# uber-research/UPSNet

Measured on AMD Instinct MI355X. Metric: images/sec (whole node), UPSNet-50 1024x2048, higher is better.
Workload: dtype f32

## Files before the change

include/upsnet_hip.h:

```cpp
#ifndef UPSNET_HIP_H
#define UPSNET_HIP_H

#include <stddef.h>
#include <stdint.h>

#ifdef __cplusplus
extern "C" {
#endif

const char *upsnet_last_error(void);
const char *upsnet_last_kernel_form(void);
int upsnet_abi_version(void);

int upsnet_zero_fill(void *stream, void *ptr, size_t bytes);


int upsnet_roi_align_forward(void *stream, const float *bottom_data, float spatial_scale, int num_rois,
                             int height, int width, int channels, int pooled_height, int pooled_width,
                             int sampling_ratio, const float *bottom_rois, float *top_data);

int upsnet_roi_align_forward_nhwc(void *stream, const float *feat_nhwc, int batch, int height, int width,
                                  int channels, float spatial_scale, const float *rois, int num_rois,
                                  int pooled_height, int pooled_width, int sampling_ratio, float *out_nhwc);

// ... 114 lines not shown

int upsnet_conv2d_nhwc_bf16(void *stream, int nseg, const float *const x[], const float *const residual[], float *const out[],
                            const int batch[], const int height[], const int width[], int Cin, const void *wpack_hi,
                            const void *wpack_lo, int ldw, const float *bias, int Cout, int KH, int KW, int stride, int pad,
                            int relu);
int upsnet_conv_pack_weight_bf16(void *stream, const float *weight, int cout, int cin, int kh, int kw, int ldw, void *wpack_hi,
                                 void *wpack_lo);
int upsnet_bottleneck_proj_bf16(void *stream, const void *x, void *out, int batch, int height_in, int width_in, int cin, int cmid, int stride,
                                const void *w1, const void *w2, const void *w3d, const float *b1, const float *b2, const float *b3d);
int upsnet_conv_bf16_tuning(int enable, int tile_rows);
int upsnet_conv1x1_bf16_tuning(int enable);
int upsnet_stem_pool_pack_weight_f32(void *stream, const float *weight, int cin, float *wpack);
int upsnet_stem_pool_f32(void *stream, const float *x4, int batch, int height, int width, const float *wpack, const float *bias, float *out);
int upsnet_stem_pool_pack_weight_bf16(void *stream, const float *weight, int cin, void *wpack);
int upsnet_stem_pool_bf16(void *stream, const float *x4, int batch, int height, int width, const void *wpack, const float *bias, void *out);
int upsnet_deconv2x2_nhwc_bf16(void *stream, const void *x, int batch, int height, int width, int Cin, const void *wpack_hi, int ldw,
                               const float *bias, int Cout, int relu, void *out, int out_bf16);

int upsnet_bottleneck_bf16(void *stream, const void *x, void *out, int batch, int height, int width, int cmid, const void *w1,
                           const void *w2, const void *w3, const float *b1, const float *b2, const float *b3);

int upsnet_conv2d_stem_nhwc4_f32(void *stream, const float *x, int batch, int height, int width, const float *wpack,
                                 int ldw, const float *bias, int Cout, int KH, int KW, int stride, int pad, int relu,
                                 float *out);
int upsnet_conv_pack_weight_stem(void *stream, const float *weight, int cout, int cin, int kh, int kw, int ldw, float *wpack);

int upsnet_deconv2x2_nhwc_f32(void *stream, const float *x, int batch, int height, int width, int Cin, const float *wpack,
                              int ldw, const float *bias, int Cout, int relu, float *out);
int upsnet_deconv2x2_pack_weight(void *stream, const float *weight, int cin, int cout, int ldw, float *wpack);

int upsnet_deconv2x2_frag_nhwc_f32(void *stream, const float *x, float *out, int batch, int height, int width, int Cin,
                                   const float *wpack, const float *bias4, int Cout, int relu);

void upsnet_conv_tuning(int winograd_tiles, int force_tile);

int upsnet_conv_pack_weight(void *stream, const float *weight, int cout, int cin, int kh, int kw, int ldw, float *wpack);

int upsnet_conv1x1_frag_nhwc_f32(void *stream, const float *x, const float *residual, float *out, int batch, int height, int width,
                                 int Cin, const float *wpack, const float *bias, int Cout, int stride, int relu, int residual_up);
void upsnet_conv1x1_tuning(int bn);
int upsnet_conv1x1_siblings_nhwc_f32(void *stream, const float *x, float *out_a, float *out_b, int batch, int height, int width, int Cin,
                                     const float *wpack, const float *bias, int cout_a, int cout_b, int stride, int relu_a, int relu_b);
void upsnet_conv1x1_pair32_tuning(int waves);

int upsnet_residency_tuning(int kernel, int cap);
size_t upsnet_residency_pad_bytes(int cap, size_t static_lds, size_t dynamic_lds);
int upsnet_residency_last_dynamic_lds(void);

int upsnet_conv2d_winograd36_nhwc_f32(void *stream, int nseg, const float *const x[], float *const out[], const int batch[],
                                      const int height[], const int width[], int Cin, const float *wpack, int ldw, const float *bias,
                                      int Cout, int relu);
int upsnet_conv_pack_weight_winograd36(void *stream, const float *weight, int cout, int cin, int ldw, float *wpack);
size_t upsnet_conv2d_winograd36_splitk_workspace_bytes(int batch, int height, int width, int Cout, int ksplit);
int upsnet_conv2d_winograd36_nhwc_f32_splitk(void *stream, const float *x, float *out, int batch, int height, int width, int Cin,
                                             const float *wpack, int ldw, const float *bias, int Cout, int relu, int ksplit, void *workspace);

size_t upsnet_conv1x1_ksw_packed_weight_floats(int cout, int cin);
int upsnet_conv1x1_ksw_pack_weight(void *stream, const float *weight, int cout, int cin, float *wpack);
int upsnet_conv1x1_ksw_nhwc_f32(void *stream, const float *x, const float *residual, float *out, int batch, int height, int width, int Cin,
                                const float *wpack, const float *bias, int Cout, int stride, int relu, int tile_pixels, int tile_channels,
                                int split_n);
void upsnet_conv1x1_ksw_tuning(int tile);

size_t upsnet_conv3x3_ksw_packed_weight_floats(int cin);
int upsnet_conv3x3_ksw_pack_weight(void *stream, const float *weight, int cout, int cin, float *wpack);
int upsnet_conv3x3_ksw_nhwc_f32(void *stream, const float *x, float *out, int batch, int height, int width, int Cin, const float *wpack,
// ... 337 lines not shown
```

upsnet_amd/_lib.py:

```python
import ctypes
import os

import torch

_HERE = os.path.dirname(os.path.abspath(__file__))
LIB_PATH = os.environ.get("UPSNET_LIB_PATH") or os.path.join(_HERE, "csrc", "libupsnet_hip.so")

c_int, c_float, c_double, c_void_p, c_size_t, c_long = ctypes.c_int, ctypes.c_float, ctypes.c_double, ctypes.c_void_p, ctypes.c_size_t, ctypes.c_long
P = c_void_p

_SIGNATURES = {
    "upsnet_last_error": (ctypes.c_char_p, []),
    "upsnet_last_kernel_form": (ctypes.c_char_p, []),
    "upsnet_abi_version": (c_int, []),
    "upsnet_zero_fill": (c_int, [P, P, c_size_t]),
    "upsnet_roi_align_forward": (c_int, [P, P, c_float, c_int, c_int, c_int, c_int, c_int, c_int, c_int, P, P]),
    "upsnet_roi_align_forward_nhwc": (c_int, [P, P, c_int, c_int, c_int, c_int, c_float, P, c_int, c_int, c_int, c_int, P]),
    "upsnet_fpn_roi_align_forward": (c_int, [P, P, P, P, P, c_int, P, c_int, P, c_int, c_int, c_int, P, P]),
    "upsnet_fpn_roi_order": (c_int, [P, P, c_int, P, c_int, c_int, P]),
    "upsnet_fpn_roi_align_forward_ordered": (c_int, [P, P, P, P, P, c_int, P, c_int, P, c_int, c_int, c_int, P, P, P]),
    "upsnet_roi_tuning": (None, [c_int]),
    "upsnet_roi_geometry": (None, [c_int, c_int]),
    "upsnet_deform_im2col": (c_int, [P, P, P] + [c_int] * 13 + [P]),
    "upsnet_mod_deform_im2col": (c_int, [P, P, P, P] + [c_int] * 15 + [P]),
# ... 36 lines not shown
    "upsnet_conv_tuning": (None, [c_int, c_int]),
    "upsnet_conv_pack_weight": (c_int, [P, P, c_int, c_int, c_int, c_int, c_int, P]),
    "upsnet_nms_host": (c_int, [P, P, P, c_int, c_int, c_float, c_int]),
    "upsnet_nms_workspace_bytes": (c_size_t, [c_int, c_int]),
    "upsnet_nms_batched": (c_int, [P, P, P, P, P, c_int, c_int, c_float, P, P, P]),
    "upsnet_nms_tuning": (None, [c_int]),
    "upsnet_cpu_nms_batched": (c_int, [P, P, P, P, c_int, c_int, c_double, P, P, P]),
    "upsnet_soft_nms_batched_workspace_bytes": (c_size_t, [c_int, c_int]),
    "upsnet_soft_nms_batched": (c_int, [P, P, P, P, c_int, c_int, c_float, c_float, c_float, c_int, P, P]),
    "upsnet_soft_nms_workspace_bytes": (c_size_t, [c_int]),
    "upsnet_soft_nms": (c_int, [P, P, P, c_int, c_float, c_float, c_float, c_int, P, P]),
    "upsnet_proposal_workspace_bytes": (c_size_t, [c_int, P, P, c_int, c_int, c_int]),
    "upsnet_pyramid_proposals_strided": (c_int, [P, c_int, P, P, P, P, P, P, P, P, P, P, c_int, P, c_int, c_int, c_float, c_float, P, P, P, P]),
    "upsnet_pyramid_proposals_strided_ordered": (c_int, [P, c_int, P, P, P, P, P, P, P, P, P, P, c_int, P, c_int, c_int, c_float, c_float, P, P, P, P, P]),
    "upsnet_pyramid_proposals_joint_strided": (c_int, [P, c_int, P, P, P, P, P, P, P, P, P, P, c_int, P, c_int, c_int, c_float, c_float, P, P, P, P]),
    "upsnet_pyramid_proposals": (c_int, [P, c_int, P, P, P, P, P, P, c_int, P, c_int, c_int, c_float, c_float, P, P, P, P]),
    "upsnet_mask_roi_capacity": (c_int, [c_int, c_int, c_int]),
    "upsnet_mask_roi_workspace_bytes": (c_size_t, [c_int, c_int, c_int]),
    "upsnet_mask_roi": (c_int, [P, P, P, P, c_int, P, c_int, P, c_int, c_float, c_float, c_int, P, P, P, P, P, P, P]),
    "upsnet_mask_roi_ex": (c_int, [P, P, P, P, c_int, P, c_int, P, c_int, c_int, c_float, c_float, c_int, P, P, P, P, P, P, P]),
    "upsnet_mask_logit_gather": (c_int, [P, P, c_int, c_int, c_int, c_long, c_long, c_long, P, P, c_int, P]),
    "upsnet_mask_removal_workspace_bytes": (c_size_t, [c_int, c_int, c_int, c_int]),
    "upsnet_mask_removal": (c_int, [P, P, P, P, P, c_int, P, c_int, c_int, c_int, c_int, c_double, P, P, P, P]),
    "upsnet_panoptic_tail_pack": (c_int, [P, P, P, c_int, P, P, P, P, P, P, P, P]),
    "upsnet_mask_paste": (c_int, [P, P, P, P, P, P, c_int, c_int, c_int, c_int, P]),
    "upsnet_seg_term": (c_int, [P, P, c_int, c_int, c_int, P, P, P, c_int, P]),
    "upsnet_panoptic_fuse": (c_int, [P, P, c_int, c_int, c_int, c_int, P, P, P, P, P, P, c_int, c_int, P, c_int, P, P]),
    "upsnet_panoptic_fuse_up": (c_int, [P, P, c_int, c_int, c_int, c_int, c_int, c_int, P, P, P, P, P, P, c_int, c_int, P, P, P]),
    "upsnet_conv2d_stem_nhwc4_f32": (c_int, [P, P, c_int, c_int, c_int, P, c_int, P, c_int, c_int, c_int, c_int, c_int, c_int, P]),
    "upsnet_conv_pack_weight_stem": (c_int, [P, P, c_int, c_int, c_int, c_int, c_int, P]),
    "upsnet_deconv2x2_nhwc_f32": (c_int, [P, P, c_int, c_int, c_int, c_int, P, c_int, P, c_int, c_int, P]),
    "upsnet_deconv2x2_pack_weight": (c_int, [P, P, c_int, c_int, c_int, P]),
    "upsnet_deconv2x2_frag_nhwc_f32": (c_int, [P, P, P, c_int, c_int, c_int, c_int, P, P, c_int, c_int]),
    "upsnet_prep_image_u8": (c_int, [P, P, c_int, c_int, P, c_double, c_int, c_int, c_int, c_int, c_int, P]),
    "upsnet_image_to_nhwc4": (c_int, [P, P, c_int, c_int, c_int, c_int, P]),
    "upsnet_unified_pan_workspace_bytes": (c_size_t, []),
    "upsnet_unified_pan_result": (c_int, [P, P, P, P, c_int, c_int, c_int, c_int, c_int, c_int, P, P]),
    "upsnet_combined_pan_workspace_bytes": (c_size_t, [c_int, c_long]),
    "upsnet_combined_pan_result": (c_int, [P, c_int, P, c_int, c_int, c_long, P, P, c_int, c_int, c_int, c_double, P]),
    "upsnet_mask_roi_dedup": (c_int, [P, P, P, P, c_int, P, P, P, P, c_int, P, P, P]),
    "upsnet_conv2d_winograd_nhwc_f32": (c_int, [P, c_int, P, P, P, P, P, P, c_int, P, c_int, P, c_int, c_int]),
    "upsnet_conv2d_winograd_nhwc_f32_splitk": (c_int, [P, P, P, P, c_int, c_int, c_int, c_int, P, c_int, P, c_int, c_int, c_int, P]),
    "upsnet_conv_pack_weight_winograd": (c_int, [P, P, c_int, c_int, c_int, P]),
    "upsnet_conv_pack_weight_winograd_tn32": (c_int, [P, P, c_int, c_int, c_int, P]),
    "upsnet_conv2d_winograd_nhwc_f32_tn32": (c_int, [P, c_int, P, P, P, P, P, P, c_int, P, c_int, P, c_int, c_int]),
    "upsnet_conv2d_winograd_nhwc_f32_tail": (c_int, [P, P, P, c_int, c_int, c_int, c_int, c_int, P, c_int, P, c_int, P, c_int, c_int]),
    "upsnet_conv2d_winograd36_nhwc_f32": (c_int, [P, c_int, P, P, P, P, P, c_int, P, c_int, P, c_int, c_int]),
    "upsnet_conv_pack_weight_winograd36": (c_int, [P, P, c_int, c_int, c_int, P]),
    "upsnet_conv2d_nhwc_bf16": (c_int, [P, c_int, P, P, P, P, P, P, c_int, P, P, c_int, P, c_int, c_int, c_int, c_int, c_int, c_int]),
    "upsnet_bottleneck_proj_bf16": (c_int, [P, P, P, c_int, c_int, c_int, c_int, c_int, c_int, P, P, P, P, P, P]),
    "upsnet_conv_bf16_tuning": (c_int, [c_int, c_int]),
    "upsnet_conv1x1_bf16_tuning": (c_int, [c_int]),
    "upsnet_stem_pool_pack_weight_f32": (c_int, [P, P, c_int, P]),
    "upsnet_stem_pool_f32": (c_int, [P, P, c_int, c_int, c_int, P, P, P]),
    "upsnet_stem_pool_pack_weight_bf16": (c_int, [P, P, c_int, P]),
    "upsnet_stem_pool_bf16": (c_int, [P, P, c_int, c_int, c_int, P, P, P]),
    "upsnet_deconv2x2_nhwc_bf16": (c_int, [P, P, c_int, c_int, c_int, c_int, P, c_int, P, c_int, c_int, P, c_int]),
    "upsnet_bottleneck_bf16": (c_int, [P, P, P, c_int, c_int, c_int, c_int, P, P, P, P, P, P]),
    "upsnet_conv_pack_weight_bf16": (c_int, [P, P, c_int, c_int, c_int, c_int, c_int, P, P]),
    "upsnet_conv2d_splitk_workspace_bytes": (c_size_t, [c_int, c_int, c_int, c_int, c_int, c_int, c_int, c_int, c_int]),
    "upsnet_conv2d_nhwc_f32_splitk": (c_int, [P, P, P, P, c_int, c_int, c_int, c_int, P, c_int, P, c_int, c_int, c_int, c_int, c_int, c_int, c_int, P]),
    "upsnet_im_post_rle": (c_int, [P, P, P, P, c_int, c_int, c_int, c_int, c_int, c_int, P, P]),
    "upsnet_fcn_score_combine": (c_int, [P, c_int, P, c_int, c_int, c_int, P, P]),
    "upsnet_panoptic_argmax": (c_int, [P, P, c_int, c_int, c_int, c_int, P, P, c_int, c_int, P]),
    "upsnet_pq_workspace_bytes": (c_size_t, [c_int]),
    "upsnet_pq_accumulate": (c_int, [P, P, P, c_int, c_int, P, c_int, P, c_int, c_int, P, P, P, P, P, P]),
# ... 140 lines not shown
```

upsnet_amd/build.py:

```python
import hashlib
import os
import re
import subprocess
import sys

HERE = os.path.dirname(os.path.abspath(__file__))
CSRC = os.path.join(HERE, "csrc")
INCLUDE = os.path.join(os.path.dirname(HERE), "include")
LIB = os.path.join(CSRC, "libupsnet_hip.so")
STAMP = LIB + ".srchash"
SOURCES = ["capi.cpp", "fill.hip", "roi_align.hip", "nms.hip", "deform_conv.hip", "deform_fused.hip", "deform_fused_bf16.hip", "backward.hip", "conv.hip", "conv1x1.hip", "conv1x1_ksw.hip", "conv1x1_pair.hip", "conv_wino.hip", "conv_wino36.hip", "conv_bf16.hip", "bottleneck_bf16.hip", "conv3x3_wreg_bf16.hip", "conv1x1_wreg_bf16.hip", "stem_pool_bf16.hip", "stem_pool.hip", "proposal.hip", "detect.hip", "panoptic.hip", "fcn_head.hip", "preprocess.hip", "postprocess.hip", "pq_eval.hip", "pq_boundary.hip", "det_eval.hip", "poly_raster.hip", "restore.hip", "pan_combine.hip", "prop_eval.hip", "cs_inst_eval.hip", "cs_pixel_eval.hip", "pan_format.hip", "vis_render.hip", "pan_vis.hip", "gt_prepare.hip", "group_norm.hip", "cs_inst_format.hip", "tta.hip", "box_vote.hip", "pan_track.hip", "video_eval.hip", "mots_eval.hip", "pan_components.hip"]
FLAGS = ["--offload-arch=gfx950", "-O3", "-ffp-contract=off", "-fno-slp-vectorize", "-std=c++17", "-fPIC", "-Wall", "-Wno-unused-function"]


_COMMENT = re.compile(rb"//[^\n]*|/\*.*?\*/", re.S)


def _source_hash():
    h = hashlib.sha1(" ".join(FLAGS + SOURCES).encode())
    deps = sorted(os.path.join(CSRC, f) for f in os.listdir(CSRC) if f.endswith((".hip", ".cpp", ".h")))
    deps.append(os.path.join(INCLUDE, "upsnet_hip.h"))
    for d in deps:
        h.update(os.path.basename(d).encode())
        with open(d, "rb") as f:
            h.update(b" ".join(_COMMENT.sub(b" ", f.read()).split()))
    return h.hexdigest()


def _stale():
    if not os.path.exists(LIB) or not os.path.exists(STAMP):
        return True
    with open(STAMP) as f:
        return f.read().strip() != _source_hash()


def build(force=False, verbose=True):
    if not force and not _stale():
        return LIB
    hipcc = os.environ.get("HIPCC", "hipcc")
    objs = []
    procs = []
    for src in SOURCES:
        obj = os.path.join(CSRC, os.path.splitext(src)[0] + ".o")
        cmd = [hipcc] + FLAGS + ["-I" + INCLUDE, "-I" + CSRC, "-x", "hip", "-c", os.path.join(CSRC, src), "-o", obj]
# ... 19 lines not shown
```

upsnet_amd/knobs.py:

```python
import os
import re

_ROOT = os.path.dirname(os.path.abspath(__file__))
_NAME = re.compile(r'UPSNET_[A-Z0-9_]+')

REGISTRY = {
    'UPSNET_ALLOW_LIBRARY_CONV': ('0', 'models/hipconv.py', 'a convolution no hand-written kernel covers runs on the library instead of raising'),
    'UPSNET_BF16_ACT': ('1', 'models/hipconv.py', 'bf16 mode: bf16 activations between the layers (0: fp32 activations)'),
    'UPSNET_BF16_BLOCK': ('1', 'models/hipconv.py', 'bf16 mode: one-launch bottlenecks (0: three launches)'),
    'UPSNET_BF16_BLOCK_MIN_TILES': ('128', 'models/hipconv.py', 'bf16 mode: fewest tiles for the one-launch bottleneck'),
    'UPSNET_BF16_HALO': ('1', 'csrc/conv_bf16.hip', 'bf16 3x3 layers on the haloed-patch kernel (0: general kernel)'),
    'UPSNET_BF16_MIN_WG': ('192', 'models/hipconv.py', 'bf16 mode: fewest workgroups for a bf16 layer'),
    'UPSNET_BF16_MIN_WG_WREG': ('16', 'models/hipconv.py', 'bf16 mode: fewest workgroups for the weights-from-L2 3x3 kernel'),
    'UPSNET_BF16_NARROW_BELOW': ('384', 'csrc/conv_bf16.hip', 'bf16 general kernel: 128 x 64 tiles below this many workgroups'),
    'UPSNET_BF16_PROJ': ('1', 'models/hipconv.py', 'bf16 mode: projection bottlenecks as one launch'),
    'UPSNET_BF16_STEM': ('1', 'models/hipconv.py', 'bf16 mode: fused stem + pool kernel'),
    'UPSNET_BF16_WREG': ('1', 'csrc/conv3x3_wreg_bf16.hip', 'bf16 3x3 layers on the weights-from-L2 kernel'),
    'UPSNET_BF16_WREG1': ('1', 'csrc/conv1x1_wreg_bf16.hip', 'bf16 1x1 layers on the no-LDS kernel where it wins'),
    'UPSNET_BF16_WREG_TH': ('auto', 'csrc/conv3x3_wreg_bf16.hip', 'tile rows of the weights-from-L2 3x3 kernel'),
    'UPSNET_CONV1X1': ('1', 'models/hipconv.py', '1x1 layers on the lean GEMM kernel (0: implicit-GEMM kernel)'),
    'UPSNET_CONV1X1_BALANCE': ('0', 'models/hipconv.py', 'split-K tail for unevenly tiled 1x1 layers'),
    'UPSNET_CONV1X1_MIN_WG': ('256', 'models/hipconv.py', 'fewest workgroups for the lean 1x1 kernel'),
    'UPSNET_CONV1X1_KSW': ('1', 'models/hipconv.py', 'small-tile (16x16x4 fragment) 1x1 kernel for maps the 64-pixel tiles do not fill evenly'),
    'UPSNET_CONV1X1_KSW_MAX_FILL': ('0.75', 'models/hipconv.py', 'use it when the last round of 64-pixel workgroups is less than this full'),
    'UPSNET_CONV3X3_KSW': ('1', 'models/hipconv.py', 'small-tile 3x3 kernel for <= 32-channel layers (offset predictors) on small maps'),
    'UPSNET_CONV1X1_PAIR': ('1', 'models/hipconv.py', 'conv3 + next conv1 in one launch'),
    'UPSNET_CONV1X1_PAIR32_WAVES': ('8', 'ops.py', 'waves per workgroup of the res4 pair kernel'),
    'UPSNET_CONV1X1_PAIR_MIN_TILES': ('1024', 'models/hipconv.py', 'fewest tiles for the res2 pair kernel'),
    'UPSNET_CONV1X1_PAIR_RES3': ('1', 'models/hipconv.py', 'pair kernel on res3'),
    'UPSNET_CONV1X1_PAIR_RES4': ('1', 'models/hipconv.py', 'pair kernel on res4'),
    'UPSNET_CONV1X1_SIBLINGS': ('1', 'models/hipconv.py', 'conv1 + projection shortcut in one launch'),
    'UPSNET_CONV_PRECISION': ('fp32', 'models/hipconv.py', 'fp32 | bf16 | bf16x3 (bench.py --conv-precision)'),
    'UPSNET_DCN_BF16': ('1', 'ops.py', 'bf16 mode: fused deformable convolution on the bf16 cores'),
    'UPSNET_DCN_KERNEL': ('frag', 'ops.py', 'generation of the fused deformable kernel'),
    'UPSNET_DCN_SMALL_GRID': ('0', 'csrc/deform_fused.hip', 'small-grid variant threshold of the fused deformable kernel'),
    'UPSNET_DCN_SPLITK': ('1', 'ops.py', 'split-K for the offset predictors of small maps'),
    'UPSNET_DCN_VARIANT': ('5', 'csrc/deform_fused.hip', 'schedule variant of the fused deformable kernel'),
    'UPSNET_DECONV_FRAG': ('1', 'models/hipconv.py', 'transposed convolution on the lean GEMM kernel'),
    'UPSNET_DIST_BACKEND': ('nccl', 'upsnet_end2end_test.py', 'torch.distributed backend of the harness (gloo when ranks share a GPU)'),
    'UPSNET_EARLY_MASK': ('1', 'models/resnet_upsnet.py', 'mask head on the side stream as soon as the detections exist'),
    'UPSNET_FC_RELU': ('1', 'models/rcnn.py', 'ReLU of fc6 / fc7 in the library GEMM epilogue (0: separate elementwise launch)'),
    'UPSNET_GRAPH': ('1', 'models/resnet_upsnet.py', 'whole forward as one HIP graph'),
    'UPSNET_GRAPH_ALIAS': ('1', 'models/resnet_upsnet.py', 'outputs are views into the graph buffers (0: copies)'),
    'UPSNET_GRAPH_OWN_STREAM': ('0', 'models/resnet_upsnet.py', 'capture / replay on an own stream with one instance'),
    'UPSNET_GRAPH_SLOTS': ('2', 'models/resnet_upsnet.py', 'graph instances per input shape'),
    'UPSNET_HIP_MEMSET': ('0', 'csrc/fill.hip', 'zero scratch with hipMemsetAsync instead of a kernel'),
    'UPSNET_LIB_PATH': ('', '_lib.py', 'path of libupsnet_hip.so (same-box A/B of two builds)'),
    'UPSNET_NMS_LDS': ('0', 'csrc/nms.hip', 'stage the suppression mask in LDS'),
    'UPSNET_NMS_SCAN16': ('1', 'csrc/nms.hip', 'unrolled scan for <= 1024 boxes'),
    'UPSNET_OVERLAP': ('1', 'models/resnet_upsnet.py', 'semantic branch on a side stream'),
    'UPSNET_PIN': ('1', 'upsnet_end2end_test.py', 'pin each rank to its CPU slice'),
    'UPSNET_ROI_KERNEL': ('auto', 'csrc/roi_align.hip', 'ROIAlign kernel variant 0..4; auto = 3 (corner-sharing) for >= 100 bins per ROI, else 0 -- so '
                                                        '"0" is NOT the default; upsnet_roi_tuning(v >= 0) overrides the variable, (v < 0) returns to it'),
    'UPSNET_ROI_XCD_ORDER': ('1', 'ops.py', 'deal the ROIs of the box head\'s ROIAlign launch to the XCDs by image neighbourhood (table written by prop_merge_kernel)'),
    'UPSNET_ROI_XCD_ORDER_MIN': ('512', 'ops.py', 'only for launches with at least this many ROIs'),
    'UPSNET_ROI_XCD_ORDER_STANDALONE': ('0', 'ops.py', 'build the table with a launch of its own for ROI sets that do not come from pyramid_proposals'),
    'UPSNET_ROI_PER_BIN': ('0', 'csrc/roi_align.hip', 'one wave per (roi, bin) (older decomposition)'),
    'UPSNET_SHARE_GPU': ('0', 'upsnet_end2end_test.py', 'let N ranks share one GPU (functional runs of the N > 1 path)'),
    'UPSNET_SPLITK': ('1', 'models/hipconv.py', 'split-K forms for small maps'),
    'UPSNET_STEM_POOL': ('1', 'models/hipconv.py', 'fused stem + pool kernel (0: stem kernel + library pool)'),
    'UPSNET_WINO36': ('1', 'models/hipconv.py', 'largest 3x3 / stride 1 layers on the Winograd F(4x4,3x3) kernel'),
    'UPSNET_WINO36_SPLITK': ('0', 'models/hipconv.py', 'res3 / res4 conv2 and FPN P4 on the split-K F(4x4) form (3-5 us per launch; more rounding error)'),
    'UPSNET_WINO36_PREFIX': ('0', 'models/hipconv.py', 'multi-map F(4x4) launches keep only the leading maps that fill whole rounds of workgroups (measured: no gain)'),
    'UPSNET_WINO36_ROI': ('1', 'models/hipconv.py', 'mask head (ROI batches) on the Winograd F(4x4,3x3) kernel (0: F(2x2) with the half-size tail)'),
    'UPSNET_WINO36_MIN_FILL': ('0.65', 'models/hipconv.py', 'F(4x4,3x3) only if its last round of workgroups is at least this full'),
    'UPSNET_WINOGRAD': ('1', 'models/hipconv.py', '3x3 / stride 1 layers on the Winograd kernel'),
    'UPSNET_WINOGRAD_MIN_WG': ('128', 'models/hipconv.py', 'fewest workgroups for the Winograd kernel'),
    'UPSNET_WINO_TAIL_FUSED': ('1', 'models/hipconv.py', 'mask-head tail inside the main launch (0: two launches)'),
    'UPSNET_WINO_TAIL_SPLIT': ('1', 'models/hipconv.py', 'mask-head tail on half-size workgroups'),
    'UPSNET_WINO_TM64_MIN': ('768', 'models/hipconv.py', '64-tile Winograd workgroups above this many'),
}


def known():
    return set(REGISTRY)


def scan_sources():
    names = set()
    files = [os.path.join(os.path.dirname(_ROOT), 'bench.py')]
# ... 23 lines not shown
```

upsnet_amd/models/hipconv.py:

```python
import collections
import os

import torch
import torch.nn as nn
import torch.nn.functional as F

from .. import group_norm, ops

ENABLED = True
ALLOW_LIBRARY = os.environ.get('UPSNET_ALLOW_LIBRARY_CONV', '0') == '1'
FALLBACKS = []
TRACE = None


def _library(m, x, why):
    if x.is_cuda:
        FALLBACKS.append((repr(m), why))
        if not ALLOW_LIBRARY:
            raise RuntimeError('upsnet_amd.hipconv: %r on a CUDA tensor %s is not covered by the hand-written kernels (%s); set '
                               'UPSNET_ALLOW_LIBRARY_CONV=1 to run it on the library convolution' % (m, tuple(x.shape), why))


def _trace(kind, **kw):
    if TRACE is not None:
# ... 668 lines not shown
    return y


DECONV_FRAG = os.environ.get('UPSNET_DECONV_FRAG', '1') != '0'


def deconv2x2(m, x, relu=False):
    geom = (ENABLED and isinstance(m, nn.ConvTranspose2d) and x.is_cuda and tuple(m.kernel_size) == (2, 2) and
            tuple(m.stride) == (2, 2) and tuple(m.padding) == (0, 0) and tuple(m.output_padding) == (0, 0) and m.groups == 1 and
            tuple(m.dilation) == (1, 1) and m.in_channels % 32 == 0)
    if geom and x.dtype == torch.bfloat16 and PRECISION == 'bf16' and m.in_channels % 64 == 0 and m.out_channels % 32 == 0:
        whi, ldw = _pack(m, 'deconv16', ops.pack_deconv2x2_weight_bf16)
        y = ops.deconv2x2_bf16(x, whi, ldw, m.bias, m.out_channels, relu=relu)
        _trace('deconv', module=m, x=x, out=y, relu=relu, form='deconv2x2 bf16')
        return y
    if x.dtype == torch.bfloat16:
        x = x.float()
    ok = geom and x.dtype == torch.float32
    if not ok:
        _library(m, x, 'not a 2x2 / stride-2 transposed convolution with Cin % 32 == 0')
        y = m(x)
        return F.relu(y, inplace=True) if relu else y
    if DECONV_FRAG and m.out_channels % 32 == 0:
        wp, bias4 = _pack(m, 'deconv_frag', lambda w: ops.pack_deconv2x2_weight_frag(w, m.bias))
        y = ops.deconv2x2_frag(x, wp, bias4, m.out_channels, relu=relu)
        _trace('deconv', module=m, x=x, out=y, relu=relu, form='deconv2x2 frag')
        return y
    wp, ldw = _pack(m, 'deconv', ops.pack_deconv2x2_weight)
    y = ops.deconv2x2(x, wp, ldw, m.bias, m.out_channels, relu=relu)
    _trace('deconv', module=m, x=x, out=y, relu=relu, form='deconv2x2')
    return y


def dcn(m, x, offset, relu=False):
    if (ENABLED and x.is_cuda and x.shape[0] == 1 and not torch.is_grad_enabled() and
            ops.fused_dcn_supported(m.in_channels, m.out_channels, m.deformable_groups, m.groups, m.padding, m.stride, m.dilation)):
        return ops.deform_conv_fused([x], [offset], ops.cached_dcn_pack(m.weight), m.bias, m.in_channels, m.out_channels, m.kernel_size,
                                     m.stride, m.padding, m.dilation, relu=relu)[0]
    y = m(x, offset)
    return torch.relu_(y) if relu else y


def head_norm(with_norm):
    assert with_norm in ['batch_norm', 'group_norm', 'none']
    if with_norm == 'batch_norm':
        raise NotImplementedError(
            "with_norm='batch_norm': the reference takes this layer from upsnet/operators/modules/distbatchnorm.py (a synchronised "
            "BatchNorm2d imported only under Horovod + syncbn), which is not part of its tree -- there is no BatchNorm2d to reproduce; "
            "use 'group_norm' or 'none'")
    return None if with_norm == 'none' else (lambda num_channels: nn.GroupNorm(32, num_channels))


def norm_supported(gn, x):
    return (ENABLED and isinstance(gn, nn.GroupNorm) and gn.affine and x.is_cuda and x.dim() in (2, 4) and x.shape[1] == gn.num_channels and
            group_norm.supported(gn.num_channels, gn.num_groups))


def _norm_library(gn, x, relu, residual, residual_up):
    _library(gn, x, 'hipconv.norm_supported() is false')
    y = gn(x)
    if residual is not None:
        y = y + (F.interpolate(residual, scale_factor=2, mode='nearest') if residual_up else residual)
    return F.relu(y, inplace=True) if relu else y


def norm(gn, x, relu=False, residual=None, residual_up=False):
# ... 29 lines not shown
```

upsnet_amd/models/rcnn.py:

```python
import os

import torch
import torch.nn as nn
import torch.nn.functional as F

from .. import ops
from ..config.config import config
from . import hipconv
from ..operators.modules.fpn_roi_align import FPNRoIAlign
from ..operators.modules.view import View


class MaskBranch(nn.Module):

    def __init__(self, num_classes, dim_in=256, dim_hidden=256, with_norm='none'):
        super(MaskBranch, self).__init__()
        norm = hipconv.head_norm(with_norm)
        self.roi_pooling = FPNRoIAlign(config.network.mask_size // 2, config.network.mask_size // 2,
                                       [1.0 / 4, 1.0 / 8, 1.0 / 16, 1.0 / 32], channels_last=True)
        if norm is not None:
            block = lambda cin: nn.Sequential(nn.Conv2d(cin, dim_hidden, 3, 1, 1, bias=False), norm(dim_hidden), nn.ReLU(inplace=True))
        else:
            block = lambda cin: nn.Sequential(nn.Conv2d(cin, dim_hidden, 3, 1, 1), nn.ReLU(inplace=True))
        self.mask_conv1 = block(dim_in)
        self.mask_conv2 = block(dim_hidden)
        self.mask_conv3 = block(dim_hidden)
        self.mask_conv4 = block(dim_hidden)
        self.mask_deconv1 = nn.Sequential(nn.ConvTranspose2d(dim_hidden, dim_hidden, 2, 2, 0), nn.ReLU(inplace=True))
        self.mask_score = nn.Conv2d(dim_hidden, num_classes, 1)
        self.initialize()

    def initialize(self):
        for m in self.modules():
            if isinstance(m, (nn.Conv2d, nn.ConvTranspose2d)):
                nn.init.kaiming_normal_(m.weight.data, mode='fan_in')
                if m.bias is not None:
                    m.bias.data.zero_()

    def forward(self, feat, rois):
        x = self.roi_pooling(feat, rois)
        for blk in (self.mask_conv1, self.mask_conv2, self.mask_conv3, self.mask_conv4):
            if len(blk) == 3:
                x = hipconv.norm(blk[1], hipconv.conv(blk[0], x, relu=False, winograd='always'), relu=True)
                continue
            x = hipconv.conv(blk[0], x, relu=True, winograd='always', out_dtype=hipconv.act_dtype())
        return hipconv.conv(self.mask_score, hipconv.deconv2x2(self.mask_deconv1[0], x, relu=True), pin=True)


FC_RELU_EPILOGUE = os.environ.get('UPSNET_FC_RELU', '1') != '0'


def _linear_relu(x, w, b):
    if FC_RELU_EPILOGUE and x.is_cuda and b is not None and x.dtype == torch.float32 and not torch.is_grad_enabled():
        return torch._addmm_activation(b, x, w.t(), use_gelu=False)
    return F.relu(F.linear(x, w, b), inplace=True)


class RCNN(nn.Module):

    def __init__(self, num_classes, num_reg_classes, pool_size=7, dim_in=256, dim_hidden=1024, with_fpn_pooling=True,
                 with_dpooling=False, with_adaptive_pooling=False, with_heavier_head=False, with_norm='none'):
        super(RCNN, self).__init__()
        assert with_fpn_pooling
        norm = hipconv.head_norm(with_norm)
        self.pool_size, self.dim_in = pool_size, dim_in
        self.roi_pooling = FPNRoIAlign(pool_size, pool_size, [1.0 / 4, 1.0 / 8, 1.0 / 16, 1.0 / 32], channels_last=True)
        if norm is not None:
            self.fc6 = nn.Sequential(nn.Linear((pool_size ** 2) * dim_in, dim_hidden), View(-1, dim_hidden, 1, 1), norm(dim_hidden),
                                     View(-1, dim_hidden), nn.ReLU(inplace=True))
        else:
            self.fc6 = nn.Sequential(nn.Linear((pool_size ** 2) * dim_in, dim_hidden), nn.ReLU(inplace=True))
        self.fc7 = nn.Sequential(nn.Linear(dim_hidden, dim_hidden), nn.ReLU(inplace=True))
        self.cls_score = nn.Linear(dim_hidden, num_classes)
        self.bbox_pred = nn.Linear(dim_hidden, num_reg_classes * 4)
        self.initialize()

    def initialize(self):
        for m in self.modules():
            if isinstance(m, nn.Linear):
# ... 26 lines not shown
```

upsnet_amd/ops.py:

```python
import os

import numpy as np
import torch

from . import _lib
from ._lib import check, f32c, float_array, int_array, lib, nhwc, ptr, ptr_array, require_cuda, stream


PROFILE = {'enabled': False, 'events': []}


def _prof_begin():
    if not PROFILE['enabled']:
        return None
    ev0 = torch.cuda.Event(enable_timing=True)
    ev0.record()
    return ev0


def _prof_end(ev0, kind, flops, nbytes, label=None):
    ev1 = torch.cuda.Event(enable_timing=True)
    ev1.record()
    PROFILE['events'].append((kind, ev0, ev1, flops, nbytes) if label is None else (kind, ev0, ev1, flops, nbytes, label))

# ... 894 lines not shown
    require_cuda(weight)
    weight = f32c(weight)
    Cin, Cout, kh, kw = weight.shape
    if (kh, kw) != (2, 2):
        raise RuntimeError("pack_deconv2x2_weight: kernel must be 2x2")
    ldw = (4 * Cout + 31) // 32 * 32
    wp = torch.empty((Cin, ldw), dtype=torch.float32, device=weight.device)
    check(lib().upsnet_deconv2x2_pack_weight(stream(), ptr(weight), Cin, Cout, ldw, ptr(wp)), "deconv2x2_pack_weight")
    return wp, ldw


def deconv2x2(x, wpack, ldw, bias, cout, relu=False):
    require_cuda(x, wpack)
    x = nhwc(x.float())
    N, C, H, W = x.shape
    out = _nhwc_out(N, cout, 2 * H, 2 * W, x.device)
    ev0 = _prof_begin()
    check(lib().upsnet_deconv2x2_nhwc_f32(stream(), ptr(x), N, H, W, C, ptr(wpack), int(ldw), ptr(None if bias is None else f32c(bias)),
                                          int(cout), int(bool(relu)), ptr(out)), "deconv2x2_nhwc_f32")
    if ev0 is not None:
        _prof_end(ev0, 'conv', 2.0 * 4 * cout * C * N * H * W, 4.0 * (C * N * H * W + 4 * cout * N * H * W + 4 * cout * C))
    return out


def pack_deconv2x2_weight_frag(weight, bias):
    require_cuda(weight)
    Cin, Cout, kh, kw = weight.shape
    if (kh, kw) != (2, 2) or Cin % 32 or Cout % 32:
        raise RuntimeError("pack_deconv2x2_weight_frag: kernel 2x2, Cin % 32 == 0, Cout % 32 == 0")
    w = weight.detach().float().permute(2, 3, 1, 0).reshape(4 * Cout, Cin, 1, 1).contiguous()
    return pack_conv1x1_weight(w), (None if bias is None else bias.detach().float().repeat(4).contiguous())


def deconv2x2_frag(x, wpack, bias4, cout, relu=False):
    require_cuda(x, wpack)
    x = nhwc(x.float())
    N, C, H, W = x.shape
    out = _nhwc_out(N, cout, 2 * H, 2 * W, x.device)
    ev0 = _prof_begin()
    check(lib().upsnet_deconv2x2_frag_nhwc_f32(stream(), ptr(x), ptr(out), N, H, W, C, ptr(wpack), ptr(bias4), int(cout), int(bool(relu))),
          "deconv2x2_frag_nhwc_f32")
    if ev0 is not None:
        _prof_end(ev0, 'conv', 2.0 * 4 * cout * C * N * H * W, 4.0 * (C * N * H * W + 4 * cout * N * H * W + 4 * cout * C),
                  "deconv 2x2/2 %d->%d [%s] (gemm)" % (C, cout, (N, H, W)))
    return out


def pack_deconv2x2_weight_bf16(weight):
    require_cuda(weight)
    Cin, Cout, kh, kw = weight.shape
    if (kh, kw) != (2, 2) or Cin % 64 or Cout % 32:
        raise RuntimeError("pack_deconv2x2_weight_bf16: kernel 2x2, Cin % 64 == 0, Cout % 32 == 0")
    w = weight.detach().float().permute(2, 3, 1, 0).reshape(4 * Cout, Cin, 1, 1).contiguous()
    hi, _, ldw = pack_conv_weight_bf16(w, split=False)
    return hi, ldw


def deconv2x2_bf16(x, whi, ldw, bias, cout, relu=False, out_dtype=torch.float32):
    require_cuda(x, whi)
    if x.dtype != torch.bfloat16:
        raise RuntimeError("deconv2x2_bf16: expects a bf16 map")
    x = nhwc(x)
    N, C, H, W = x.shape
    out16 = out_dtype == torch.bfloat16
    out = (torch.empty((N, 2 * H, 2 * W, cout), dtype=torch.bfloat16, device=x.device).permute(0, 3, 1, 2) if out16
           else _nhwc_out(N, cout, 2 * H, 2 * W, x.device))
    ev0 = _prof_begin()
    check(lib().upsnet_deconv2x2_nhwc_bf16(stream(), ptr(x), N, H, W, C, ptr(whi), int(ldw), ptr(None if bias is None else f32c(bias)),
                                           int(cout), int(bool(relu)), ptr(out), int(out16)), "deconv2x2_nhwc_bf16")
    if ev0 is not None:
        _prof_end(ev0, 'conv_bf16', 2.0 * 4 * cout * C * N * H * W,
                  2.0 * C * N * H * W + (2.0 if out16 else 4.0) * 4 * cout * N * H * W + 2.0 * 4 * cout * C)
    return out


def prep_image_u8(image_hwc, pixel_means, im_scale, resized_hw, padded_hw, nhwc4=True):
    import ctypes
    require_cuda(image_hwc)
# ... 930 lines not shown
```

Baseline: 173.3.

## Fuse mask-head 2x2 deconvolution, ReLU and 1x1 score conv into one kernel

Result: no change. 173.6 (median of 6 runs) (+0.2%).

```diff
diff --git a/include/upsnet_hip.h b/include/upsnet_hip.h
--- a/include/upsnet_hip.h
+++ b/include/upsnet_hip.h
@@ -170,6 +170,9 @@
 int upsnet_deconv2x2_frag_nhwc_f32(void *stream, const float *x, float *out, int batch, int height, int width, int Cin,
                                    const float *wpack, const float *bias4, int Cout, int relu);
 
+int upsnet_deconv2x2_score_nhwc_f32(void *stream, const float *x, float *out1, float *out, int batch, int height, int width, int Cin,
+                                    const float *w1pack, const float *bias4, const float *w2pack, const float *bias2, int Cout);
+
 void upsnet_conv_tuning(int winograd_tiles, int force_tile);
 
 int upsnet_conv_pack_weight(void *stream, const float *weight, int cout, int cin, int kh, int kw, int ldw, float *wpack);
diff --git a/upsnet_amd/_lib.py b/upsnet_amd/_lib.py
--- a/upsnet_amd/_lib.py
+++ b/upsnet_amd/_lib.py
@@ -92,6 +92,7 @@
     "upsnet_deconv2x2_nhwc_f32": (c_int, [P, P, c_int, c_int, c_int, c_int, P, c_int, P, c_int, c_int, P]),
     "upsnet_deconv2x2_pack_weight": (c_int, [P, P, c_int, c_int, c_int, P]),
     "upsnet_deconv2x2_frag_nhwc_f32": (c_int, [P, P, P, c_int, c_int, c_int, c_int, P, P, c_int, c_int]),
+    "upsnet_deconv2x2_score_nhwc_f32": (c_int, [P, P, P, P, c_int, c_int, c_int, c_int, P, P, P, P, c_int]),
     "upsnet_prep_image_u8": (c_int, [P, P, c_int, c_int, P, c_double, c_int, c_int, c_int, c_int, c_int, P]),
     "upsnet_image_to_nhwc4": (c_int, [P, P, c_int, c_int, c_int, c_int, P]),
     "upsnet_unified_pan_workspace_bytes": (c_size_t, []),
diff --git a/upsnet_amd/build.py b/upsnet_amd/build.py
--- a/upsnet_amd/build.py
+++ b/upsnet_amd/build.py
@@ -9,7 +9,7 @@
 INCLUDE = os.path.join(os.path.dirname(HERE), "include")
 LIB = os.path.join(CSRC, "libupsnet_hip.so")
 STAMP = LIB + ".srchash"
-SOURCES = ["capi.cpp", "fill.hip", "roi_align.hip", "nms.hip", "deform_conv.hip", "deform_fused.hip", "deform_fused_bf16.hip", "backward.hip", "conv.hip", "conv1x1.hip", "conv1x1_ksw.hip", "conv1x1_pair.hip", "conv_wino.hip", "conv_wino36.hip", "conv_bf16.hip", "bottleneck_bf16.hip", "conv3x3_wreg_bf16.hip", "conv1x1_wreg_bf16.hip", "stem_pool_bf16.hip", "stem_pool.hip", "proposal.hip", "detect.hip", "panoptic.hip", "fcn_head.hip", "preprocess.hip", "postprocess.hip", "pq_eval.hip", "pq_boundary.hip", "det_eval.hip", "poly_raster.hip", "restore.hip", "pan_combine.hip", "prop_eval.hip", "cs_inst_eval.hip", "cs_pixel_eval.hip", "pan_format.hip", "vis_render.hip", "pan_vis.hip", "gt_prepare.hip", "group_norm.hip", "cs_inst_format.hip", "tta.hip", "box_vote.hip", "pan_track.hip", "video_eval.hip", "mots_eval.hip", "pan_components.hip"]
+SOURCES = ["capi.cpp", "fill.hip", "roi_align.hip", "nms.hip", "deform_conv.hip", "deform_fused.hip", "deform_fused_bf16.hip", "backward.hip", "conv.hip", "conv1x1.hip", "conv1x1_ksw.hip", "conv1x1_pair.hip", "deconv_score.hip", "conv_wino.hip", "conv_wino36.hip", "conv_bf16.hip", "bottleneck_bf16.hip", "conv3x3_wreg_bf16.hip", "conv1x1_wreg_bf16.hip", "stem_pool_bf16.hip", "stem_pool.hip", "proposal.hip", "detect.hip", "panoptic.hip", "fcn_head.hip", "preprocess.hip", "postprocess.hip", "pq_eval.hip", "pq_boundary.hip", "det_eval.hip", "poly_raster.hip", "restore.hip", "pan_combine.hip", "prop_eval.hip", "cs_inst_eval.hip", "cs_pixel_eval.hip", "pan_format.hip", "vis_render.hip", "pan_vis.hip", "gt_prepare.hip", "group_norm.hip", "cs_inst_format.hip", "tta.hip", "box_vote.hip", "pan_track.hip", "video_eval.hip", "mots_eval.hip", "pan_components.hip"]
 FLAGS = ["--offload-arch=gfx950", "-O3", "-ffp-contract=off", "-fno-slp-vectorize", "-std=c++17", "-fPIC", "-Wall", "-Wno-unused-function"]
 
 
diff --git a/upsnet_amd/csrc/deconv_score.hip b/upsnet_amd/csrc/deconv_score.hip
--- /dev/null
+++ b/upsnet_amd/csrc/deconv_score.hip
@@ -0,0 +1,235 @@
+#include "conv_params.h"
+#include "upsnet_hip.h"
+
+typedef unsigned uintx4 __attribute__((ext_vector_type(4)));
+typedef float floatx4 __attribute__((ext_vector_type(4)));
+
+#define DS_PITCH 65
+#define DS_CMID 256
+
+struct DeconvScoreParams {
+    const float *x, *w1, *b1, *w2, *b2;
+    float *out1, *out;
+    long M;
+    int H, W, Cin, Cout;
+    int tiles;
+};
+
+static inline size_t ds_tile_bytes(int Cin)
+{
+    const int quarters = Cin / 4 > DS_CMID / 4 ? Cin / 4 : DS_CMID / 4;
+    return (size_t)quarters * DS_PITCH * 16;
+}
+
+template <int NC, bool STORE1>
+__global__ void __launch_bounds__(512, 2) deconv_score_f32_kernel(const DeconvScoreParams p)
+{
+    constexpr int NPART = NC == 16 ? 2 : 4;
+    constexpr int LDP = NC + 4;
+    extern __shared__ __attribute__((aligned(16))) unsigned char smem_raw[];
+    const int nsl = p.Cin >> 5;
+    const int quarters = max(8 * nsl, DS_CMID / 4);
+    float4 *Xs = reinterpret_cast<float4 *>(smem_raw);
+    float *Ysf = reinterpret_cast<float *>(smem_raw);
+    float *red = reinterpret_cast<float *>(smem_raw);
+    unsigned *rowoff = reinterpret_cast<unsigned *>(Xs + quarters * DS_PITCH);
+    const int tid = threadIdx.x, lane = tid & 63;
+    const int wave = __builtin_amdgcn_readfirstlane(tid >> 6);
+    const int lhalf = lane >> 5, l32 = lane & 31;
+    const int bid = (int)blockIdx.x;
+    const int dydx = (bid >> 3) & 3, tile = (bid & 7) + 8 * (bid >> 5);
+    if (tile >= p.tiles) return;
+    const int dy = dydx >> 1, dx = dydx & 1;
+    const long p0 = (long)tile * 64;
+
+    if (tid < 64) {
+        const long pp = p0 + tid;
+        unsigned o = 0x80000000u;
+        if (pp < p.M) {
+            const long HW = (long)p.H * p.W;
+            const int n = (int)(pp / HW);
+            const int rem = (int)(pp - (long)n * HW);
+            const int h = rem / p.W, w = rem - h * p.W;
+            o = (unsigned)((n * 2 * p.H + 2 * h + dy) * 2 * p.W + 2 * w + dx);
+        }
+        rowoff[tid] = o;
+    }
+
+#define DS_RSRC(NAME, PTR, BYTES)                                                                                      \
+    const size_t NAME##_a = reinterpret_cast<size_t>(PTR);                                                             \
+    const __amdgpu_buffer_rsrc_t NAME = __builtin_amdgcn_make_buffer_rsrc(                                             \
+        reinterpret_cast<void *>(((size_t)(unsigned)__builtin_amdgcn_readfirstlane((unsigned)(NAME##_a >> 32)) << 32) |  \
+                                 (size_t)(unsigned)__builtin_amdgcn_readfirstlane((unsigned)NAME##_a)), 0, (int)(BYTES), 0x00020000);
+    DS_RSRC(xrsrc, p.x, __builtin_amdgcn_readfirstlane((unsigned)(p.M * p.Cin) * 4u))
+    DS_RSRC(w1rsrc, reinterpret_cast<const char *>(p.w1) + (size_t)(dydx * 8 + wave) * (size_t)nsl * 4096u, nsl * 4096)
+    DS_RSRC(w2rsrc, p.w2, NC * DS_CMID * 4)
+    DS_RSRC(o1rsrc, p.out1, STORE1 ? __builtin_amdgcn_readfirstlane((unsigned)p.M * (4u * DS_CMID * 4u)) : 0u)
+#undef DS_RSRC
+    const unsigned b_lane = (unsigned)(lhalf * 512 + l32 * 16);
+    const int gmax = 4 * nsl - 1;
+#define DS_LD(D, RS, VO, SO) { const uintx4 v_ = __builtin_amdgcn_raw_buffer_load_b128(RS, (VO), (SO), 0); \
+        D = make_float4(__uint_as_float(v_.x), __uint_as_float(v_.y), __uint_as_float(v_.z), __uint_as_float(v_.w)); }
+#define DS_B1(SLOT, G) DS_LD(b1r[SLOT], w1rsrc, b_lane, (unsigned)min((G), gmax) * 1024u)
+
+    float4 b1r[4];
+    {
+        const int q = tid & 7, prow = tid >> 3;
+        const long pp = p0 + prow;
+        const unsigned po = pp < p.M ? (unsigned)pp * 4u * (unsigned)p.Cin + 16u * (unsigned)q : 0x80000000u;
+        for (int s0 = 0; s0 < nsl; s0 += 8) {
+            float4 xa[8];
+#pragma unroll
+            for (int s = 0; s < 8; ++s) DS_LD(xa[s], xrsrc, s0 + s < nsl ? po + 128u * (unsigned)(s0 + s) : 0x80000000u, 0)
+            if (s0 == 0) {
+#pragma unroll
+                for (int u = 0; u < 4; ++u) DS_B1(u, u)
+            }
+#pragma unroll
+            for (int s = 0; s < 8; ++s)
+                if (s0 + s < nsl) Xs[(8 * (s0 + s) + q) * DS_PITCH + prow] = xa[s];
+        }
+    }
+    __syncthreads();
+
+    floatx16 acc0, acc1;
+#pragma unroll
+    for (int r = 0; r < 16; ++r) { acc0[r] = 0.f; acc1[r] = 0.f; }
+    {
+        const float4 *xfrag = Xs + lhalf * DS_PITCH + l32;
+        float4 a0 = xfrag[0], a1 = xfrag[32];
+        for (int s = 0; s < nsl; ++s) {
+#pragma unroll
+            for (int u = 0; u < 4; ++u) {
+                const float4 *nx = xfrag + 2 * min(4 * s + u + 1, gmax) * DS_PITCH;
+                const float4 n0 = nx[0], n1 = nx[32];
+                const float4 bf = b1r[u];
+                __builtin_amdgcn_sched_barrier(0);
+                acc0 = __builtin_amdgcn_mfma_f32_32x32x2f32(a0.x, bf.x, acc0, 0, 0, 0);
+                acc1 = __builtin_amdgcn_mfma_f32_32x32x2f32(a1.x, bf.x, acc1, 0, 0, 0);
+                acc0 = __builtin_amdgcn_mfma_f32_32x32x2f32(a0.y, bf.y, acc0, 0, 0, 0);
+                acc1 = __builtin_amdgcn_mfma_f32_32x32x2f32(a1.y, bf.y, acc1, 0, 0, 0);
+                acc0 = __builtin_amdgcn_mfma_f32_32x32x2f32(a0.z, bf.z, acc0, 0, 0, 0);
+                acc1 = __builtin_amdgcn_mfma_f32_32x32x2f32(a1.z, bf.z, acc1, 0, 0, 0);
+                acc0 = __builtin_amdgcn_mfma_f32_32x32x2f32(a0.w, bf.w, acc0, 0, 0, 0);
+                acc1 = __builtin_amdgcn_mfma_f32_32x32x2f32(a1.w, bf.w, acc1, 0, 0, 0);
+                DS_B1(u, 4 * s + u + 4)
+                a0 = n0; a1 = n1;
+                __builtin_amdgcn_sched_barrier(0);
+            }
+        }
+    }
+#undef DS_B1
+    const int part = NC == 16 ? (wave >> 2) : (wave >> 1);
+    float4 b2r[8];
+#pragma unroll
+    for (int t = 0; t < 8; ++t) DS_LD(b2r[t], w2rsrc, (unsigned)lane * 16u, (unsigned)(part * 8 + t) * 1024u)
+#undef DS_LD
+    __syncthreads();
+
+    {
+        const int c = 32 * wave + l32;
+        const float bv = p.b1 != nullptr ? p.b1[dydx * DS_CMID + c] : 0.f;
+        float *ydst = Ysf + ((c >> 2) * DS_PITCH + 4 * lhalf) * 4 + (c & 3);
+#pragma unroll
+        for (int i = 0; i < 2; ++i) {
+#pragma unroll
+            for (int k4 = 0; k4 < 4; ++k4) {
+                unsigned rr4[4] = {0u, 0u, 0u, 0u};
+                if (STORE1) {
+                    const uintx4 ro = *reinterpret_cast<const uintx4 *>(rowoff + 32 * i + 8 * k4 + 4 * lhalf);
+                    rr4[0] = ro.x; rr4[1] = ro.y; rr4[2] = ro.z; rr4[3] = ro.w;
+                }
+#pragma unroll
+                for (int j = 0; j < 4; ++j) {
+                    const int r = 4 * k4 + j;
+                    float v = i == 0 ? acc0[r] : acc1[r];
+                    if (p.b1 != nullptr) v = v + bv;
+                    v = fmaxf(v, 0.f);
+                    if (STORE1)
+                        __builtin_amdgcn_raw_buffer_store_b32(__float_as_uint(v), o1rsrc, (rr4[j] * (DS_CMID * 4u) + 4u * (unsigned)c) | (rr4[j] & 0x80000000u), 0, 0);
+                    ydst[(32 * i + 8 * k4 + j) * 4] = v;
+                }
+            }
+        }
+    }
+    __syncthreads();
+
+    const float4 *Ys = Xs;
+    if constexpr (NC == 16) {
+        const int rb = wave & 3, lk = lane >> 4, li = lane & 15;
+        const float4 *yf = Ys + (32 * part + lk) * DS_PITCH + 16 * rb + li;
+        floatx4 d = {0.f, 0.f, 0.f, 0.f};
+#pragma unroll
+        for (int t = 0; t < 8; ++t) {
+            const float4 a = yf[4 * t * DS_PITCH];
+            d = __builtin_amdgcn_mfma_f32_16x16x4f32(a.x, b2r[t].x, d, 0, 0, 0);
+            d = __builtin_amdgcn_mfma_f32_16x16x4f32(a.y, b2r[t].y, d, 0, 0, 0);
+            d = __builtin_amdgcn_mfma_f32_16x16x4f32(a.z, b2r[t].z, d, 0, 0, 0);
+            d = __builtin_amdgcn_mfma_f32_16x16x4f32(a.w, b2r[t].w, d, 0, 0, 0);
+        }
+        __syncthreads();
+#pragma unroll
+        for (int r = 0; r < 4; ++r) red[(part * 64 + 16 * rb + 4 * lk + r) * LDP + li] = d[r];
+    } else {
+        const int rb = wave & 1;
+        const float4 *yf = Ys + (16 * part + lhalf) * DS_PITCH + 32 * rb + l32;
+        floatx16 d;
+#pragma unroll
+        for (int r = 0; r < 16; ++r) d[r] = 0.f;
+#pragma unroll
+        for (int t = 0; t < 8; ++t) {
+            const float4 a = yf[2 * t * DS_PITCH];
+            d = __builtin_amdgcn_mfma_f32_32x32x2f32(a.x, b2r[t].x, d, 0, 0, 0);
+            d = __builtin_amdgcn_mfma_f32_32x32x2f32(a.y, b2r[t].y, d, 0, 0, 0);
+            d = __builtin_amdgcn_mfma_f32_32x32x2f32(a.z, b2r[t].z, d, 0, 0, 0);
+            d = __builtin_amdgcn_mfma_f32_32x32x2f32(a.w, b2r[t].w, d, 0, 0, 0);
+        }
+        __syncthreads();
+#pragma unroll
+        for (int r = 0; r < 16; ++r) red[(part * 64 + 32 * rb + 8 * (r >> 2) + 4 * lhalf + (r & 3)) * LDP + l32] = d[r];
+    }
+    __syncthreads();
+
+#pragma unroll
+    for (int e = tid; e < 64 * NC; e += 512) {
+        const int pix = e / NC, col = e - pix * NC;
+        float v = red[pix * LDP + col] + red[(64 + pix) * LDP + col];
+        if (NPART == 4) v = v + (red[(128 + pix) * LDP + col] + red[(192 + pix) * LDP + col]);
+        const unsigned o = rowoff[pix];
+        if (col < p.Cout && !(o & 0x80000000u)) {
+            if (p.b2 != nullptr) v = v + p.b2[col];
+            p.out[(size_t)o * (size_t)p.Cout + col] = v;
+        }
+    }
+}
+
+extern "C" int upsnet_deconv2x2_score_nhwc_f32(void *stream, const float *x, float *out1, float *out, int batch, int height, int width, int Cin,
+                                               const float *w1pack, const float *bias4, const float *w2pack, const float *bias2, int Cout)
+{
+    UPS_REQUIRE(x && out && w1pack && w2pack && batch > 0 && height > 0 && width > 0, "deconv2x2_score_nhwc_f32: null pointer / empty map");
+    UPS_REQUIRE(Cin > 0 && Cin % 32 == 0 && Cin <= 512, "deconv2x2_score_nhwc_f32: Cin must be a multiple of 32, at most 512 (got %d)", Cin);
+    UPS_REQUIRE(Cout >= 1 && Cout <= 32, "deconv2x2_score_nhwc_f32: 1 <= Cout <= 32 (got %d)", Cout);
+    const long M = (long)batch * height * width;
+    UPS_REQUIRE(M * Cin < (1L << 29) && M * 4 * DS_CMID < (1L << 29), "deconv2x2_score_nhwc_f32: feature map exceeds 2 GiB; split the batch");
+    DeconvScoreParams p;
+    p.x = x; p.w1 = w1pack; p.b1 = bias4; p.w2 = w2pack; p.b2 = bias2; p.out1 = out1; p.out = out;
+    p.M = M; p.H = height; p.W = width; p.Cin = Cin; p.Cout = Cout;
+    p.tiles = (int)((M + 63) / 64);
+    const size_t smem = ds_tile_bytes(Cin) + 64 * sizeof(unsigned);
+    static std::atomic<unsigned long long> attr_dev{0};
+#define DS_ATTR(NC, S1) UPS_CHECK_HIP(hipFuncSetAttribute(reinterpret_cast<const void *>(&deconv_score_f32_kernel<NC, S1>), hipFuncAttributeMaxDynamicSharedMemorySize, 163840))
+    UPS_ONCE_PER_DEVICE(attr_dev, DS_ATTR(16, false); DS_ATTR(16, true); DS_ATTR(32, false); DS_ATTR(32, true));
+#undef DS_ATTR
+    const dim3 grid((unsigned)(32 * ((p.tiles + 7) / 8)));
+    hipStream_t st = (hipStream_t)stream;
+    if (Cout <= 16) {
+        if (out1) hipLaunchKernelGGL((deconv_score_f32_kernel<16, true>), grid, dim3(512), smem, st, p);
+        else hipLaunchKernelGGL((deconv_score_f32_kernel<16, false>), grid, dim3(512), smem, st, p);
+    } else {
+        if (out1) hipLaunchKernelGGL((deconv_score_f32_kernel<32, true>), grid, dim3(512), smem, st, p);
+        else hipLaunchKernelGGL((deconv_score_f32_kernel<32, false>), grid, dim3(512), smem, st, p);
+    }
+    UPS_CHECK_LAUNCH("deconv_score_f32_kernel");
+    ups_set_form("deconv_score<%d,%d>", Cout <= 16 ? 16 : 32, out1 ? 1 : 0);
+    return 0;
+}
diff --git a/upsnet_amd/knobs.py b/upsnet_amd/knobs.py
--- a/upsnet_amd/knobs.py
+++ b/upsnet_amd/knobs.py
@@ -46,6 +46,7 @@
     'UPSNET_GRAPH_SLOTS': ('2', 'models/resnet_upsnet.py', 'graph instances per input shape'),
     'UPSNET_HIP_MEMSET': ('0', 'csrc/fill.hip', 'zero scratch with hipMemsetAsync instead of a kernel'),
     'UPSNET_LIB_PATH': ('', '_lib.py', 'path of libupsnet_hip.so (same-box A/B of two builds)'),
+    'UPSNET_MASK_TAIL': ('1', 'models/hipconv.py', 'mask head: transposed convolution + ReLU + score in one launch (0: two launches)'),
     'UPSNET_NMS_LDS': ('0', 'csrc/nms.hip', 'stage the suppression mask in LDS'),
     'UPSNET_NMS_SCAN16': ('1', 'csrc/nms.hip', 'unrolled scan for <= 1024 boxes'),
     'UPSNET_OVERLAP': ('1', 'models/resnet_upsnet.py', 'semantic branch on a side stream'),
diff --git a/upsnet_amd/models/hipconv.py b/upsnet_amd/models/hipconv.py
--- a/upsnet_amd/models/hipconv.py
+++ b/upsnet_amd/models/hipconv.py
@@ -724,6 +724,35 @@
     return y
 
 
+MASK_TAIL = os.environ.get('UPSNET_MASK_TAIL', '1') != '0'
+
+
+def use_deconv_score(deconv, score, x):
+    if not (MASK_TAIL and DECONV_FRAG and ENABLED and PRECISION == 'fp32' and x.is_cuda and x.dtype == torch.float32):
+        return False
+    if not (isinstance(deconv, nn.ConvTranspose2d) and tuple(deconv.kernel_size) == (2, 2) and tuple(deconv.stride) == (2, 2) and
+            tuple(deconv.padding) == (0, 0) and tuple(deconv.output_padding) == (0, 0) and deconv.groups == 1 and
+            tuple(deconv.dilation) == (1, 1) and deconv.in_channels % 32 == 0 and deconv.in_channels <= 512 and deconv.out_channels == 256):
+        return False
+    if not (isinstance(score, nn.Conv2d) and _plain(score, 1, 0) and score.in_channels == 256 and score.out_channels <= 32 and
+            score.padding_mode == 'zeros'):
+        return False
+    return x.shape[0] * x.shape[2] * x.shape[3] * max(deconv.in_channels, 1024) < (1 << 29)
+
+
+def deconv2x2_score(deconv, score, x):
+    if not use_deconv_score(deconv, score, x):
+        return conv(score, deconv2x2(deconv, x, relu=True), pin=True)
+    w1, bias4 = _pack(deconv, 'deconv_frag', lambda w: ops.pack_deconv2x2_weight_frag(w, deconv.bias))
+    w2 = _pack(score, 'deconv_score', ops.pack_deconv_score_weight)
+    if TRACE is None:
+        return ops.deconv2x2_frag(x, w1, bias4, deconv.out_channels, relu=True, score=(w2, score.bias, score.out_channels))
+    y, mid = ops.deconv2x2_frag(x, w1, bias4, deconv.out_channels, relu=True, score=(w2, score.bias, score.out_channels), keep_deconv=True)
+    _trace('deconv', module=deconv, x=x, out=mid, relu=True, form='deconv2x2 + score (deconv)')
+    _trace('conv', module=score, x=mid, out=y, relu=False, residual=None, residual_up=False, form='igemm in deconv2x2 + score')
+    return y
+
+
 def dcn(m, x, offset, relu=False):
     if (ENABLED and x.is_cuda and x.shape[0] == 1 and not torch.is_grad_enabled() and
             ops.fused_dcn_supported(m.in_channels, m.out_channels, m.deformable_groups, m.groups, m.padding, m.stride, m.dilation)):
diff --git a/upsnet_amd/models/rcnn.py b/upsnet_amd/models/rcnn.py
--- a/upsnet_amd/models/rcnn.py
+++ b/upsnet_amd/models/rcnn.py
@@ -44,7 +44,7 @@
                 x = hipconv.norm(blk[1], hipconv.conv(blk[0], x, relu=False, winograd='always'), relu=True)
                 continue
             x = hipconv.conv(blk[0], x, relu=True, winograd='always', out_dtype=hipconv.act_dtype())
-        return hipconv.conv(self.mask_score, hipconv.deconv2x2(self.mask_deconv1[0], x, relu=True), pin=True)
+        return hipconv.deconv2x2_score(self.mask_deconv1[0], self.mask_score, x)
 
 
 FC_RELU_EPILOGUE = os.environ.get('UPSNET_FC_RELU', '1') != '0'
diff --git a/upsnet_amd/ops.py b/upsnet_amd/ops.py
--- a/upsnet_amd/ops.py
+++ b/upsnet_amd/ops.py
@@ -950,10 +950,25 @@
     return pack_conv1x1_weight(w), (None if bias is None else bias.detach().float().repeat(4).contiguous())
 
 
-def deconv2x2_frag(x, wpack, bias4, cout, relu=False):
+def deconv2x2_frag(x, wpack, bias4, cout, relu=False, score=None, keep_deconv=False):
     require_cuda(x, wpack)
     x = nhwc(x.float())
     N, C, H, W = x.shape
+    if score is not None:
+        w2pack, bias2, cout2 = score
+        if cout != 256 or not relu:
+            raise RuntimeError("deconv2x2_frag: the fused score needs 256 deconvolution channels and the ReLU")
+        require_cuda(w2pack)
+        logits = _nhwc_out(N, cout2, 2 * H, 2 * W, x.device)
+        mid = _nhwc_out(N, cout, 2 * H, 2 * W, x.device) if keep_deconv else None
+        ev0 = _prof_begin()
+        check(lib().upsnet_deconv2x2_score_nhwc_f32(stream(), ptr(x), ptr(mid), ptr(logits), N, H, W, C, ptr(wpack), ptr(bias4), ptr(w2pack),
+                                                    ptr(None if bias2 is None else f32c(bias2)), int(cout2)), "deconv2x2_score_nhwc_f32")
+        if ev0 is not None:
+            _prof_end(ev0, 'conv', 2.0 * 4 * (cout * C + cout2 * cout) * N * H * W,
+                      4.0 * (C * N * H * W + 4 * cout2 * N * H * W + 4 * cout * C + cout2 * cout),
+                      "deconv 2x2/2 %d->%d + score 1x1 ->%d [%s] (gemm)" % (C, cout, cout2, (N, H, W)))
+        return (logits, mid) if keep_deconv else logits
     out = _nhwc_out(N, cout, 2 * H, 2 * W, x.device)
     ev0 = _prof_begin()
     check(lib().upsnet_deconv2x2_frag_nhwc_f32(stream(), ptr(x), ptr(out), N, H, W, C, ptr(wpack), ptr(bias4), int(cout), int(bool(relu))),
@@ -962,6 +977,18 @@
         _prof_end(ev0, 'conv', 2.0 * 4 * cout * C * N * H * W, 4.0 * (C * N * H * W + 4 * cout * N * H * W + 4 * cout * C),
                   "deconv 2x2/2 %d->%d [%s] (gemm)" % (C, cout, (N, H, W)))
     return out
+
+
+def pack_deconv_score_weight(weight):
+    require_cuda(weight)
+    cout, cmid = weight.shape[0], weight.shape[1]
+    if cmid != 256 or not 1 <= cout <= 32 or tuple(weight.shape[2:]) != (1, 1):
+        raise RuntimeError("pack_deconv_score_weight: a [Cout <= 32, 256, 1, 1] weight")
+    nc = 16 if cout <= 16 else 32
+    parts, groups = (2, 4) if nc == 16 else (4, 2)
+    w = torch.zeros((nc, cmid), dtype=torch.float32, device=weight.device)
+    w[:cout] = weight.detach().float().reshape(cout, cmid)
+    return w.view(nc, parts, 8, groups, 4).permute(1, 2, 3, 0, 4).contiguous().view(-1)
 
 
 def pack_deconv2x2_weight_bf16(weight):
```
